# EspressoSystems/Push-CDN

Measured on AMD Instinct MI355X. Metric: broadcast_msgs_per_sec, higher is better.
Workload: dtype uint8; 1 GPU; model=gpu-broker-mesh, payload_bytes=1024, subscribers_total=10000, subscribers_per_broker=10000, topics=8, mode=broadcast, population=all, drops=0, parallelism=single-broker, global_batch=256, seq_len=1024

## Files before the change

### csrc/common/tick_geom.h

```cpp
#pragma once

#include <stdint.h>

#define K2B_BLK 32

#define DENSE_THREADS 256
#define DENSE_MAX_V 8
#define DENSE_GROUP 8
struct DenseGeom { int32_t n_chunks; int32_t chunk_units; };
static inline DenseGeom dense_geom(int32_t units_per_rec) {
    const int32_t cap = DENSE_THREADS * DENSE_MAX_V;
    const int32_t image = units_per_rec * K2B_BLK;
    DenseGeom g;
    g.n_chunks = (image + cap - 1) / cap;
    g.chunk_units = ((image + g.n_chunks - 1) / g.n_chunks + 63) & ~63;
    return g;
}
static inline int64_t dense_grid_x(int32_t n_users, int32_t group, int32_t n_chunks) {
    return ((int64_t)n_users + group - 1) / group * n_chunks;
}

static inline int64_t k2b_blocks(int64_t M) { return (M + K2B_BLK - 1) / K2B_BLK; }
static inline int64_t uniform_tick_scratch64(int64_t M, int64_t W, int64_t units_per_rec) {
    return 4 * M + W * M + k2b_blocks(M) * W * 64 + W * 64 + 2 * M * units_per_rec;
}
static inline int64_t uniform_tick_scratch32(int64_t M, int64_t W) {
    return 3 * M + 3 * k2b_blocks(M) * W * 64 + 2 * W * 64;
}
```

### csrc/gpu_bindings.cpp

```cpp

#include <torch/extension.h>
#include <ATen/hip/HIPContext.h>
#include <c10/core/DeviceGuard.h>
#include <hip/hip_runtime.h>

#include <cstdint>

#include "hip/bls_kernels.h"
#include "hip/dataplane.h"

template <typename T> struct Stored { using type = T; };
template <> struct Stored<uint64_t> { using type = int64_t; };
template <> struct Stored<uint32_t> { using type = int32_t; };
template <> struct Stored<PairRec> { using type = int32_t; };

struct Shape { int64_t dim = -1, rows = -1, cols = -1; };
static constexpr Shape vec() { return {1, -1, -1}; }
static constexpr Shape mat(int64_t rows = -1, int64_t cols = -1) { return {2, rows, cols}; }

class Op {
public:
    enum Where { kDevice, kPinnedHost };

    explicit Op(const char* name) : name_(name) {}
// ... 650 lines not shown
    t.M = a.i32(M, "M");
    t.hash_seed = hash_seed;
    t.sub_bitmap = a.ptr<uint64_t>(sub_bitmap, "sub_bitmap", 0, mat(256, -1));
    const int64_t W = sub_bitmap.size(1);
    t.W = a.i32(W, "W");
    t.n_users = a.i32(n_users, "n_users", 0, W * 64);
    a.ring_bytes(ring_bytes);
    t.ring_bytes = ring_bytes;
    t.ring_wpos = a.ptr<uint64_t>(ring_wpos, "ring_wpos", n_users);
    t.pairs = a.pairs(pairs);
    t.capacity = a.i32(pairs.size(0), "pair capacity");
    t.drops = a.ptr<uint32_t>(drops, "drops", 1);
    t.n_pairs = a.ptr<int32_t>(n_pairs, "n_pairs", 1);
    t.n_sparse = a.ptr<int32_t>(n_sparse, "n_sparse", 1);
    t.scratch64 = a.ptr<int64_t>(scratch64, "scratch64", uniform_tick_scratch64(M, W, rec / 16));
    t.scratch32 = a.ptr<int32_t>(scratch32, "scratch32", uniform_tick_scratch32(M, W));
    t.egress = a.ptr<uint8_t>(egress, "egress", n_users * ring_bytes);
    t.seq_base = (uint32_t)seq_base;
    t.nt = nt != 0;
    t.dense = dense != 0;
    TORCH_CHECK(buf.numel() >= M * uniform_len, a.name(), ": buf has ", buf.numel(),
                " bytes, shorter than M = ", M, " messages of uniform_len = ", uniform_len);
    check_flat_shape(pairs, rec / 16);
    TORCH_CHECK(M * (rec / 16) < (int64_t(1) << 31)
                && dense_grid_x(t.n_users, DENSE_GROUP, dense_geom((int32_t)(rec / 16)).n_chunks)
                       * k2b_blocks(M) < (int64_t(1) << 31),
                a.name(), ": batch too large for the dense fan-out");
    TORCH_CHECK((uintptr_t)t.scratch64 % 16 == 0, a.name(), ": scratch64 must be 16-byte aligned");
    hipStream_t s = a.begin();
    if (M == 0) return;
    launch_tick_uniform_broadcast(&t, s);
    a.launched();
}

std::vector<int64_t> uniform_tick_scratch_sizes(int64_t M, int64_t W, int64_t rec) {
    return {uniform_tick_scratch64(M, W, rec / 16), uniform_tick_scratch32(M, W)};
}

void drain_cursors(torch::Tensor ring_wpos, torch::Tensor staging, torch::Tensor host) {
    Op a("drain_cursors");
    int64_t* wpos = a.ptr<int64_t>(ring_wpos, "ring_wpos");
    const int32_t n = a.i32(ring_wpos.numel(), "cursor count");
    int64_t* st = a.ptr<int64_t>(staging, "staging", n);
    int64_t* h = a.ptr<int64_t>(host, "host", n, {}, Op::kPinnedHost);
    hipStream_t s = a.begin();
    if (n == 0) return;
    launch_drain_cursors(wpos, st, n, s);
    a.launched();
    a.check(hipMemcpyAsync(h, st, (size_t)n * 8, hipMemcpyDeviceToHost, s), "copy");
    a.check(hipStreamSynchronize(s), "sync");
}

PYBIND11_MODULE(TORCH_EXTENSION_NAME, m) {
    m.def("tick_uniform_broadcast", &tick_uniform_broadcast,
          "fused uniform broadcast tick: K4, K2a, K2b tiles, dense + sparse fan-out");
    m.def("uniform_tick_scratch_sizes", &uniform_tick_scratch_sizes,
          "(int64, int32) scratch elements tick_uniform_broadcast needs for (M, W, rec)");
    m.def("drain_cursors", &drain_cursors,
          "fused drain: cursors -> pinned host buffer, cursors zeroed, stream synchronised",
          py::call_guard<py::gil_scoped_release>());
    m.def("topic_mask_origin_t", &topic_mask_origin_t,
          "K2a transposed with per-message origin: remote-origin rows keep user bits only");
    m.def("emit_direct_peers", &emit_direct_peers,
          "K5b with peer recipient slots (owner -(p+2) -> ring n_users+p, local origin only)");
    m.def("direct_apply", &direct_apply,
          "K6: batched DirectMap upserts/deletes on the device table");
    m.def("parse_batch", &parse_batch, "K4: on-device capnp parse of a message batch",
          py::arg("buf"), py::arg("offsets"), py::arg("hash_seed") = 0);
    m.def("topic_mask", &topic_mask, "K2a: per-message subscriber mask");
    m.def("assign_emit", &assign_emit, "K2b: per-user FIFO ring assignment + pair list");
    m.def("fanout", &fanout, "K3: N-way payload fan-out into egress rings");
    m.def("direct_lookup", &direct_lookup, "K5: batched direct-route hash probe");
    m.def("apply_subs", &apply_subs, "K2c: apply subscribe/unsubscribe batch to bitmap");
    m.def("bls_verify_batch", &bls_verify_batch, "K1: batched BLS-over-BN254 verification");
    m.def("compact_rings", &compact_rings,
          "K7: gather used egress-ring prefixes into one staging buffer");
    m.def("precompute_g2_lines", &precompute_g2_lines,
          "fixed-g2 Miller line coefficients for K1 v2 (once per process)");
    m.def("bls_verify_batch2", &bls_verify_batch2,
          "K1 v2: 2-lane Fp2-decomposed batched BLS verification");
    m.def("bls_verify_batch_wave", &bls_verify_batch_wave,
          "K1 v3: wave-batched product verification (shared final exp, "
          "exact per-item fallback)");
    m.def("hash_to_g1_batch", &hash_to_g1_batch, "K1 helper: batched hash-to-G1");
    m.def("fanout_wave", &fanout_wave, "K3v2: wave-per-pair fan-out (nt flag, device count)");
    m.def("fanout_ref", &fanout_ref,
          "K3r: fan-out with by-reference records at or above ref_threshold");
    m.def("fanout_flat2", &fanout_flat2, "K3v4: flat fan-out, seq from base, capacity clamp");
    m.def("fanout_flat3", &fanout_flat3, "K3v5: graph-capturable (device seq counter)");
    m.def("seq_advance", &seq_advance, "bump the device seq counter (inside the graph)");
    m.def("topic_mask_t", &topic_mask_t, "K2a transposed: mask[W][M]");
    m.def("emit_direct", &emit_direct,
          "K5b: on-device direct-delivery pair emission (no host sync)");
    m.def("assign_emit_fused_t", &assign_emit_fused_t,
          "K2b fused on transposed mask (wave-aggregated claims, uniform-rec fast path)");
    m.def("assign_emit_blocks_t", &assign_emit_blocks_t,
          "K2b block-parallel (P1 count / P2 bases / P3 emit) for uniform records");
}
```

### csrc/hip/dataplane.hip

```cpp

#include <hip/hip_runtime.h>
#include <stdint.h>

#include "../common/divmagic.h"
#include "dataplane.h"

#define WAVE 64
#ifndef CDN_CHECK
#define CDN_CHECK 1
#endif

#define RING_ALIGN 16ull
__host__ __device__ inline uint64_t ring_rec(int32_t len) {
    return ((uint64_t)len + 16 + (RING_ALIGN - 1)) & ~(RING_ALIGN - 1);
}

typedef unsigned int cdn_v4u __attribute__((ext_vector_type(4)));
template <int NT>
__device__ __forceinline__ void store16(void* dst, cdn_v4u v) {
    if (NT) __builtin_nontemporal_store(v, (cdn_v4u*)dst);
    else *(cdn_v4u*)dst = v;
}

__device__ __forceinline__ void store_pair(PairRec* p, int32_t u, int32_t m, int64_t d) {
// ... 2 lines not shown
    store16<0>(p, v);
}

__host__ __device__ inline uint64_t fnv1a64(const uint8_t* data, uint32_t len,
                                            uint64_t seed = 0) {
    uint64_t h = 0xcbf29ce484222325ull ^ seed;
    for (uint32_t i = 0; i < len; ++i) {
        h ^= (uint64_t)data[i];
        h *= 0x100000001b3ull;
    }
    return h;
}


__device__ inline uint64_t ld_u64(const uint8_t* p) {
    uint64_t v;
    memcpy(&v, p, 8);
    return v;
}

__device__ inline bool read_struct_ptr(const uint8_t* seg, int64_t nwords, int64_t pw,
                                       int64_t* tgt, int32_t* dw, int32_t* ptrw) {
    if (pw < 0 || pw >= nwords) return false;
    uint64_t v = ld_u64(seg + pw * 8);
    if (v == 0 || (v & 3) != 0) return false;
    int64_t b = (v >> 2) & 0x3fffffff;
    if (b & 0x20000000) b -= 0x40000000;
    int32_t d = (v >> 32) & 0xffff;
    int32_t p = (v >> 48) & 0xffff;
    int64_t t = pw + 1 + b;
    if (t < 0 || t + d + p > nwords) return false;
    *tgt = t; *dw = d; *ptrw = p;
    return true;
}

__device__ inline bool read_byte_list(const uint8_t* seg, int64_t nwords, int64_t pw,
                                      int64_t* off, int32_t* len) {
    if (pw < 0 || pw >= nwords) return false;
    uint64_t v = ld_u64(seg + pw * 8);
    if (v == 0) { *off = pw; *len = 0; return true; }
    if ((v & 3) != 1) return false;
    int64_t b = (v >> 2) & 0x3fffffff;
    if (b & 0x20000000) b -= 0x40000000;
    uint32_t code = (v >> 32) & 7;
    int64_t count = (v >> 35) & 0x1fffffff;
    if (code != 2) return false;
    int64_t t = pw + 1 + b;
    if (t < 0 || t * 8 + count > nwords * 8) return false;
    *off = t * 8;
    *len = (int32_t)count;
    return true;
}

extern "C" __global__ void k4_parse_batch(
    const uint8_t* __restrict__ buf,
    const int64_t* __restrict__ offsets,
    int32_t M, uint64_t hash_seed, ParseOut out)
{
    int i = blockIdx.x * blockDim.x + threadIdx.x;
    if (i >= M) return;
    out.disc[i] = -1;
    out.payload_off[i] = 0; out.payload_len[i] = 0;
    out.topics_off[i] = 0;  out.topics_cnt[i] = 0;
    out.recip_hash[i] = 0;  out.timestamp[i] = 0;
    int64_t o_poff = 0, o_toff = 0, o_ts = 0;
    uint64_t o_rhash = 0;
    int32_t o_plen = 0, o_tcnt = 0;

    int64_t beg = offsets[i], end = offsets[i + 1];
    if (end - beg < 8 + 8) return;
    const uint8_t* p = buf + beg;
    uint32_t seg_m1, nw;
    memcpy(&seg_m1, p, 4); memcpy(&nw, p + 4, 4);
    if (seg_m1 != 0) return;
    if (8 + (int64_t)nw * 8 > end - beg) return;
    const uint8_t* seg = p + 8;
    int64_t nwords = nw;

    int64_t mt; int32_t mdw, mpw;
    if (!read_struct_ptr(seg, nwords, 0, &mt, &mdw, &mpw)) return;
    if (mdw < 1 || mpw < 1) return;
    uint16_t disc;
    memcpy(&disc, seg + mt * 8, 2);
    int64_t up = mt + mdw;

    int64_t seg_base = (seg - buf);

    switch (disc) {
    case 0: {
        int64_t it; int32_t idw, ipw;
        if (!read_struct_ptr(seg, nwords, up, &it, &idw, &ipw)) return;
        if (idw < 1 || ipw < 2) return;
        o_ts = (int64_t)ld_u64(seg + it * 8);
        int64_t ko; int32_t kl;
        if (!read_byte_list(seg, nwords, it + idw, &ko, &kl)) return;
        o_poff = kl ? seg_base + ko : 0;
        o_plen = kl;
        int64_t so; int32_t sl;
        if (!read_byte_list(seg, nwords, it + idw + 1, &so, &sl)) return;
        o_toff = sl ? seg_base + so : 0;
        o_tcnt = sl;
        break;
    }
    case 1: {
        int64_t it; int32_t idw, ipw;
        if (!read_struct_ptr(seg, nwords, up, &it, &idw, &ipw)) return;
        if (idw < 1) return;
        o_ts = (int64_t)ld_u64(seg + it * 8);
        break;
    }
    case 2: {
        int64_t it; int32_t idw, ipw;
        if (!read_struct_ptr(seg, nwords, up, &it, &idw, &ipw)) return;
        if (idw < 1 || ipw < 1) return;
        o_ts = (int64_t)ld_u64(seg + it * 8);
        int64_t co; int32_t cl;
        if (!read_byte_list(seg, nwords, it + idw, &co, &cl)) return;
        o_poff = cl ? seg_base + co : 0; o_plen = cl;
        break;
    }
    case 3: {
        int64_t it; int32_t idw, ipw;
        if (!read_struct_ptr(seg, nwords, up, &it, &idw, &ipw)) return;
        if (ipw < 2) return;
        int64_t ro; int32_t rl;
        if (!read_byte_list(seg, nwords, it + idw, &ro, &rl)) return;
        o_rhash = fnv1a64(seg + ro, rl, hash_seed);
        int64_t mo; int32_t ml;
        if (!read_byte_list(seg, nwords, it + idw + 1, &mo, &ml)) return;
        o_poff = ml ? seg_base + mo : 0; o_plen = ml;
        break;
    }
    case 4: {
        int64_t it; int32_t idw, ipw;
        if (!read_struct_ptr(seg, nwords, up, &it, &idw, &ipw)) return;
        if (ipw < 2) return;
        int64_t to; int32_t tc;
        if (!read_byte_list(seg, nwords, it + idw, &to, &tc)) return;
        o_toff = tc ? seg_base + to : 0; o_tcnt = tc;
        int64_t mo; int32_t ml;
        if (!read_byte_list(seg, nwords, it + idw + 1, &mo, &ml)) return;
        o_poff = ml ? seg_base + mo : 0; o_plen = ml;
        break;
    }
    case 5: case 6: {
        int64_t to; int32_t tc;
        if (!read_byte_list(seg, nwords, up, &to, &tc)) return;
        o_toff = tc ? seg_base + to : 0; o_tcnt = tc;
        break;
    }
    case 7: case 8: {
        int64_t dof; int32_t dl;
        if (!read_byte_list(seg, nwords, up, &dof, &dl)) return;
        o_poff = dl ? seg_base + dof : 0; o_plen = dl;
        break;
    }
    default:
        return;
    }
    out.payload_off[i] = o_poff; out.payload_len[i] = o_plen;
    out.topics_off[i] = o_toff;  out.topics_cnt[i] = o_tcnt;
    out.recip_hash[i] = (int64_t)o_rhash; out.timestamp[i] = o_ts;
    out.disc[i] = (int32_t)disc;
}


__device__ __forceinline__ uint64_t user_bits_of_word(int32_t w, int32_t n_users) {
    const int64_t lo = (int64_t)w * 64;
    if ((int64_t)n_users >= lo + 64) return ~0ull;
    if ((int64_t)n_users <= lo) return 0ull;
    return (1ull << (n_users - lo)) - 1ull;
}

template <bool SINGLE_HOP>
__device__ __forceinline__ uint64_t topic_row_or(
    const uint64_t* __restrict__ sub_bitmap, const uint8_t* __restrict__ buf,
    const int64_t* __restrict__ topics_off, const int32_t* __restrict__ topics_cnt,
    const int32_t* __restrict__ disc, int64_t m, int w, int32_t W,
    const int32_t* __restrict__ origin, int32_t n_users)
{
    uint64_t acc = 0;
    if (disc[m] == 4) {
        const uint8_t* topics = buf + topics_off[m];
        int n = topics_cnt[m];
        for (int t = 0; t < n; ++t) acc |= sub_bitmap[(int64_t)topics[t] * W + w];
        if (SINGLE_HOP && origin[m] != 0) acc &= user_bits_of_word(w, n_users);
    }
    return acc;
}

extern "C" __global__ void k2a_topic_mask(
    const uint64_t* __restrict__ sub_bitmap,
    const uint8_t* __restrict__ buf,
    const int64_t* __restrict__ topics_off,
    const int32_t* __restrict__ topics_cnt,
    const int32_t* __restrict__ disc,
    uint64_t* __restrict__ mask,
    int32_t M, int32_t W)
{
    int64_t idx = (int64_t)blockIdx.x * blockDim.x + threadIdx.x;
    if (idx >= (int64_t)M * W) return;
    int m = idx / W;
    int w = idx % W;
    mask[idx] = topic_row_or<false>(sub_bitmap, buf, topics_off, topics_cnt, disc, m, w, W,
                                    nullptr, 0);
}

extern "C" __global__ void k2b_count(
    const uint64_t* __restrict__ mask,
    int32_t M, int32_t W, int32_t n_users,
    int32_t* __restrict__ counts)
{
    int u = blockIdx.x * blockDim.x + threadIdx.x;
    if (u >= n_users) return;
    int w = u >> 6;
    uint64_t bit = 1ull << (u & 63);
// ... 470 lines not shown
        const int32_t fit = (int32_t)((ring_bytes - wpos) / (uint64_t)uniform_rec);
        uint32_t dropped = 0;
        int emitted = 0;
        const int64_t dst_base = (int64_t)u * ring_bytes + (int64_t)wpos;
        for (int m = 0; m < M; ++m) {
            if (!(col[m] & bit)) continue;
            const bool ok = (emitted < fit) && (slot < capacity);
            if (!ok) {
                if (slot < capacity) { store_pair(pairs + slot, -1, m, 0); slot++; }
                dropped++;
                continue;
            }
            store_pair(pairs + slot, u, m, dst_base + (int64_t)emitted * uniform_rec);
            slot++;
            emitted++;
        }
        ring_wpos[u] = wpos + (uint64_t)emitted * uniform_rec;
        if (dropped) atomicAdd(drops, dropped);
        return;
    }

    uint64_t wpos = ring_wpos[u];
    uint32_t dropped = 0;
    for (int m = 0; m < M; ++m) {
        if (!(col[m] & bit)) continue;
        int32_t len = payload_len[m];
        uint64_t rec = ring_rec(len);
        bool fits_ring = (wpos + rec <= (uint64_t)ring_bytes);
        bool fits_cap = (slot < capacity);
        if (!fits_ring || !fits_cap) {
            if (fits_cap) { store_pair(pairs + slot, -1, m, 0); slot++; }
            dropped++;
            continue;
        }
        store_pair(pairs + slot, u, m, (int64_t)u * ring_bytes + wpos);
        slot++;
        wpos += rec;
    }
    ring_wpos[u] = wpos;
    if (dropped) atomicAdd(drops, dropped);
}

extern "C" {

void launch_k2a_topic_mask_t(const uint64_t* sub_bitmap, const uint8_t* buf,
                             const int64_t* topics_off, const int32_t* topics_cnt,
                             const int32_t* disc, uint64_t* mask_t, int32_t M, int32_t W,
                             hipStream_t s) {
    if (M <= 0) return;
    hipLaunchKernelGGL(k2a_topic_mask_t, k2a_grid(M, W), dim3(K2A_THREADS), 0, s, sub_bitmap,
                       buf, topics_off, topics_cnt, disc, mask_t, M, W);
}


__device__ __forceinline__ void k2b_p1_body(
    const uint64_t* __restrict__ mask_t,
    int32_t M, int32_t W, int32_t NB,
    int32_t* __restrict__ bcount)
{
    const int wave = (blockIdx.x * blockDim.x + threadIdx.x) >> 6;
    if (wave >= W * NB) return;
    const int w = wave / NB, b = wave - (int64_t)(wave / NB) * NB;
    const int lane = threadIdx.x & 63;
    const uint64_t bit = 1ull << lane;
    const uint64_t* col = mask_t + (int64_t)w * M;
    const int m0 = b * K2B_BLK, m1 = min(M, m0 + K2B_BLK);
    int c = 0;
    for (int m = m0; m < m1; ++m) c += (col[m] & bit) ? 1 : 0;
    bcount[(int64_t)b * (W * 64) + (w * 64 + lane)] = c;
}

extern "C" __global__ void k2b_p1_count(
    const uint64_t* __restrict__ mask_t, int32_t M, int32_t W, int32_t NB,
    int32_t* __restrict__ bcount)
{
    k2b_p1_body(mask_t, M, W, NB, bcount);
}

struct K2bUser { int32_t base; int32_t fit; int64_t dst; };

__device__ __forceinline__ K2bUser k2b_p2_body(
    const int32_t* __restrict__ bcount,
    int u, bool active, int32_t W, int32_t NB,
    int64_t ring_bytes, int32_t capacity, int32_t uniform_rec,
    uint64_t* __restrict__ ring_wpos,
    int32_t* __restrict__ n_pairs,
    int32_t* __restrict__ pprefix,
    uint32_t* __restrict__ drops)
{
    const int lane = threadIdx.x & 63;
    int total = 0;
    if (active) {
        for (int b = 0; b < NB; ++b) {
            pprefix[(int64_t)b * (W * 64) + u] = total;
            total += bcount[(int64_t)b * (W * 64) + u];
        }
    }
    K2bUser r{wave_claim_span(total, n_pairs), 0, 0};
    uint32_t dropped = 0;
    if (active) {
        const uint64_t wpos = ring_wpos[u];
        r.fit = (int32_t)((ring_bytes - wpos) / (uint64_t)uniform_rec);
        r.dst = (int64_t)u * ring_bytes + (int64_t)wpos;
        int cap_room = capacity - r.base; if (cap_room < 0) cap_room = 0;
        int emitted = total; if (emitted > r.fit) emitted = r.fit; if (emitted > cap_room) emitted = cap_room;
        ring_wpos[u] = wpos + (uint64_t)emitted * uniform_rec;
        dropped = (uint32_t)(total - emitted);
    }
    for (int d = 1; d < 64; d <<= 1) dropped += __shfl_down(dropped, d);
    if (lane == 0 && dropped) atomicAdd(drops, dropped);
    return r;
}

extern "C" __global__ void k2b_p2_bases(
    const int32_t* __restrict__ bcount,
    int32_t W, int32_t NB, int32_t n_users,
    int64_t ring_bytes, int32_t capacity, int32_t uniform_rec,
    uint64_t* __restrict__ ring_wpos,
    int32_t* __restrict__ n_pairs,
    int32_t* __restrict__ pprefix,
    int32_t* __restrict__ ubase,
    int32_t* __restrict__ ufit,
    int64_t* __restrict__ udst,
    uint32_t* __restrict__ drops)
{
    const int u = blockIdx.x * blockDim.x + threadIdx.x;
    const bool active = u < n_users;
    const K2bUser r = k2b_p2_body(bcount, u, active, W, NB, ring_bytes, capacity, uniform_rec,
                                  ring_wpos, n_pairs, pprefix, drops);
    if (active) {
        ubase[u] = r.base;
        ufit[u] = r.fit;
        udst[u] = r.dst;
    }
}

extern "C" __global__ void k2b_p3_emit(
    const uint64_t* __restrict__ mask_t,
    const int32_t* __restrict__ pprefix,
    const int32_t* __restrict__ ubase,
    const int32_t* __restrict__ ufit,
    const int64_t* __restrict__ udst,
    int32_t M, int32_t W, int32_t NB, int32_t n_users,
    int32_t capacity, int32_t uniform_rec,
    PairRec* __restrict__ pairs)
{
    const int wave = (blockIdx.x * blockDim.x + threadIdx.x) >> 6;
    if (wave >= W * NB) return;
    const int w = wave / NB, b = wave - (int64_t)(wave / NB) * NB;
    const int lane = threadIdx.x & 63;
    const int u = w * 64 + lane;
    if (u >= n_users) return;
    const uint64_t bit = 1ull << lane;
    const uint64_t* col = mask_t + (int64_t)w * M;
    int p = pprefix[(int64_t)b * (W * 64) + u];
    const int base = ubase[u], fit = ufit[u];
    const int64_t dstb = udst[u];
    const int m0 = b * K2B_BLK, m1 = min(M, m0 + K2B_BLK);
    for (int m = m0; m < m1; ++m) {
        if (!(col[m] & bit)) continue;
        const int slot = base + p;
        if (slot < capacity) {
            if (p < fit)
                store_pair(pairs + slot, u, m, dstb + (int64_t)p * uniform_rec);
            else
                store_pair(pairs + slot, -1, m, 0);
        }
        p++;
    }
}

extern "C" void launch_k2b_blocks_t(
    const uint64_t* mask_t, int32_t M, int32_t W, int32_t n_users,
    int64_t ring_bytes, int32_t capacity, int32_t uniform_rec,
    uint64_t* ring_wpos, int32_t* n_pairs,
    int32_t* bcount, int32_t* pprefix, int32_t* ubase, int32_t* ufit, int64_t* udst,
    PairRec* pairs,
    uint32_t* drops, hipStream_t s) {
    if (M <= 0) return;
    const int NB = (M + K2B_BLK - 1) / K2B_BLK;
    const int waves = W * NB;
    const int threads = 256;
    const int blocks_wb = (waves * 64 + threads - 1) / threads;
    const int blocks_u = (n_users + threads - 1) / threads;
    hipLaunchKernelGGL(k2b_p1_count, dim3(blocks_wb), dim3(threads), 0, s,
                       mask_t, M, W, NB, bcount);
    hipLaunchKernelGGL(k2b_p2_bases, dim3(blocks_u), dim3(threads), 0, s,
                       bcount, W, NB, n_users, ring_bytes, capacity, uniform_rec,
                       ring_wpos, n_pairs, pprefix, ubase, ufit, udst, drops);
    hipLaunchKernelGGL(k2b_p3_emit, dim3(blocks_wb), dim3(threads), 0, s,
                       mask_t, pprefix, ubase, ufit, udst, M, W, NB, n_users,
                       capacity, uniform_rec, pairs);
}

void launch_k2b_fused_t(const uint64_t* mask_t, const int32_t* payload_len, int32_t M,
                        int32_t W, int32_t n_users, int64_t ring_bytes, int32_t capacity,
                        int32_t uniform_rec, uint64_t* ring_wpos, int32_t* n_pairs,
                        PairRec* pairs,
                        uint32_t* drops, hipStream_t s) {
    int threads = 256, blocks = (n_users + threads - 1) / threads;
    hipLaunchKernelGGL(k2b_fused_t, dim3(blocks), dim3(threads), 0, s, mask_t, payload_len, M,
                       W, n_users, ring_bytes, capacity, uniform_rec, ring_wpos, n_pairs,
                       pairs, drops);
}

}


__device__ __forceinline__ void k5b_claim_emit(
    int u, int i, int32_t len, int64_t ring_bytes, int32_t capacity,
    uint64_t* __restrict__ ring_wpos, int32_t* __restrict__ n_pairs,
    PairRec* __restrict__ pairs, uint32_t* __restrict__ drops)
{
    uint64_t rec = ring_rec(len);
    int slot = atomicAdd(n_pairs, 1);
    if (slot >= capacity) {
        atomicAdd(drops, 1u);
        return;
    }
    unsigned long long cur = atomicAdd((unsigned long long*)&ring_wpos[u], 0ull);
    while (true) {
        if (cur + rec > (uint64_t)ring_bytes) {
            store_pair(pairs + slot, -1, i, 0);
            atomicAdd(drops, 1u);
            return;
        }
        unsigned long long prev = atomicCAS((unsigned long long*)&ring_wpos[u], cur,
                                            cur + (unsigned long long)rec);
        if (prev == cur) break;
        cur = prev;
    }
    store_pair(pairs + slot, u, i, (int64_t)u * ring_bytes + (int64_t)cur);
}

extern "C" __global__ void k5b_emit_direct(
    const int32_t* __restrict__ disc,
    const int32_t* __restrict__ owner,
    const int64_t* __restrict__ payload_off,
    const int32_t* __restrict__ payload_len,
    int32_t M,
    int64_t ring_bytes, int32_t capacity,
    uint64_t* __restrict__ ring_wpos,
    int32_t* __restrict__ n_pairs,
    PairRec* __restrict__ pairs,
    uint32_t* __restrict__ drops)
{
    int i = blockIdx.x * blockDim.x + threadIdx.x;
// ... 137 lines not shown
                                             __HIP_MEMORY_SCOPE_AGENT);
        if (k == key) { table_vals[slot] = INT32_MIN; return; }
        if (k == 0) return;
    }
}

extern "C" {

void launch_k2a_topic_mask_origin_t(const uint64_t* sub_bitmap, const uint8_t* buf,
                                    const int64_t* topics_off, const int32_t* topics_cnt,
                                    const int32_t* disc, const int32_t* origin,
                                    uint64_t* mask_t, int32_t M, int32_t W, int32_t n_users,
                                    hipStream_t s) {
    if (M <= 0) return;
    hipLaunchKernelGGL(k2a_topic_mask_origin_t, k2a_grid(M, W), dim3(K2A_THREADS), 0, s,
                       sub_bitmap, buf, topics_off, topics_cnt, disc, origin, mask_t, M, W,
                       n_users);
}

void launch_k5b_emit_direct_peers(
    const int32_t* disc, const int32_t* owner, const int32_t* origin,
    const int64_t* payload_off, const int32_t* payload_len, int32_t M, int32_t n_users,
    int32_t n_peers, int64_t ring_bytes, int32_t capacity, uint64_t* ring_wpos,
    int32_t* n_pairs, PairRec* pairs, uint32_t* drops, hipStream_t s) {
    if (M <= 0) return;
    int threads = 256, blocks = (M + threads - 1) / threads;
    hipLaunchKernelGGL(k5b_emit_direct_peers, dim3(blocks), dim3(threads), 0, s, disc, owner,
                       origin, payload_off, payload_len, M, n_users, n_peers, ring_bytes,
                       capacity, ring_wpos, n_pairs, pairs, drops);
}

void launch_k6_direct_apply(uint64_t* table_keys, int32_t* table_vals, int64_t table_size,
                            const uint64_t* up_keys, const int32_t* up_owners, int32_t n_up,
                            const uint64_t* del_keys, int32_t n_del, uint32_t* n_failed,
                            hipStream_t s) {
    const int total = n_up + n_del;
    if (total <= 0) return;
    int threads = 256, blocks = (total + threads - 1) / threads;
    hipLaunchKernelGGL(k6_direct_apply, dim3(blocks), dim3(threads), 0, s, table_keys,
                       table_vals, table_size, up_keys, up_owners, n_up, del_keys, n_del,
                       n_failed);
}

}

extern "C" __global__ void k2b_p1_count_z(
    const uint64_t* __restrict__ mask_t, int32_t M, int32_t W, int32_t NB,
    int32_t* __restrict__ bcount, int32_t* __restrict__ n_pairs, int32_t* __restrict__ n_sparse)
{
    if (blockIdx.x == 0 && threadIdx.x == 0) { *n_pairs = 0; *n_sparse = 0; }
    k2b_p1_body(mask_t, M, W, NB, bcount);
}

extern "C" __global__ void k2b_p2_tiles(
    const int32_t* __restrict__ bcount,
    int32_t M, int32_t W, int32_t NB, int32_t n_users,
    int64_t ring_bytes, int32_t capacity, int32_t uniform_rec, int32_t use_dense,
    uint64_t* __restrict__ ring_wpos,
    int32_t* __restrict__ n_pairs,
    int32_t* __restrict__ n_sparse,
    int32_t* __restrict__ pprefix,
    int32_t* __restrict__ tslot,
    int64_t* __restrict__ tdst,
    int32_t* __restrict__ ulim,
    int32_t* __restrict__ usbase,
    int64_t* __restrict__ udst,
    uint32_t* __restrict__ drops)
{
    const int u = blockIdx.x * blockDim.x + threadIdx.x;
    const bool active = u < n_users;
    const K2bUser r = k2b_p2_body(bcount, u, active, W, NB, ring_bytes, capacity, uniform_rec,
                                  ring_wpos, n_pairs, pprefix, drops);
    int cap_room = capacity - r.base; if (cap_room < 0) cap_room = 0;
    const int lim = r.fit < cap_room ? r.fit : cap_room;
    int n_sp = 0;
    if (active) {
        int p = 0;
        for (int b = 0; b < NB; ++b) {
            const int64_t i = (int64_t)b * (W * 64) + u;
            const int cnt = bcount[i];
            const int nm = min(M - b * K2B_BLK, K2B_BLK);
            const bool dense = use_dense && cnt == nm && p + cnt <= lim;
            tdst[i] = dense ? r.dst + (int64_t)p * uniform_rec : -1;
            tslot[i] = n_sp;
            if (!dense) n_sp += max(0, min(cnt, lim - p));
            p += cnt;
        }
    }
    const int sbase = wave_claim_span(n_sp, n_sparse);
    if (active) {
        ulim[u] = lim;
        usbase[u] = sbase;
        udst[u] = r.dst;
    }
}

extern "C" __global__ void k2b_p3_sparse(
    const uint64_t* __restrict__ mask_t,
    const int32_t* __restrict__ bcount,
    const int32_t* __restrict__ pprefix,
    const int32_t* __restrict__ tslot,
    const int64_t* __restrict__ tdst,
    const int32_t* __restrict__ ulim,
    const int32_t* __restrict__ usbase,
    const int64_t* __restrict__ udst,
    int32_t M, int32_t W, int32_t NB, int32_t n_users, int32_t uniform_rec,
    PairRec* __restrict__ pairs)
{
    const int wave = (blockIdx.x * blockDim.x + threadIdx.x) >> 6;
    if (wave >= W * NB) return;
    const int w = wave / NB, b = wave - (wave / NB) * NB;
    const int lane = threadIdx.x & 63;
    const int u = w * 64 + lane;
    int p0 = 0, lim = 0, slot0 = 0;
    int64_t dstb = 0;
    bool sparse = false;
    if (u < n_users) {
        const int64_t i = (int64_t)b * (W * 64) + u;
        p0 = pprefix[i];
        lim = ulim[u];
        sparse = tdst[i] < 0 && bcount[i] > 0 && p0 < lim;
        slot0 = usbase[u] + tslot[i];
        dstb = udst[u];
    }
    unsigned long long todo = __ballot(sparse);
    if (!todo) return;
    const int m0 = b * K2B_BLK, nm = min(M - m0, K2B_BLK);
    const uint64_t word = lane < nm ? mask_t[(int64_t)w * M + m0 + lane] : 0ull;
    while (todo) {
        const int j = __ffsll((long long)todo) - 1;
        todo &= todo - 1;
        const int jp0 = __shfl(p0, j), jlim = __shfl(lim, j), jslot = __shfl(slot0, j);
        const int64_t jdst = ((int64_t)__shfl((int)(dstb >> 32), j) << 32)
                             | (uint32_t)__shfl((int)dstb, j);
        const bool bit = (word >> j) & 1ull;
        const unsigned long long mb = __ballot(bit);
        const int rank = __popcll(mb & ((1ull << lane) - 1ull));
        const int p = jp0 + rank;
        if (bit && p < jlim)
            store_pair(pairs + jslot + rank, w * 64 + j, m0 + lane,
                       jdst + (int64_t)p * uniform_rec);
    }
}

extern "C" __global__ void k3d_image(
    const uint8_t* __restrict__ buf,
    const int64_t* __restrict__ offsets,
    int32_t M, int32_t units_per_rec, uint32_t div_magic, int32_t div_shift,
    int32_t uniform_len, uint32_t seq_base,
    cdn_v4u* __restrict__ image)
{
    const uint32_t i = blockIdx.x * blockDim.x + threadIdx.x;
    if (i >= (uint32_t)(M * units_per_rec)) return;
    const int m = (int)(((uint64_t)i * div_magic) >> div_shift);
    const int q = (int)i - m * units_per_rec;
    image[i] = q == 0 ? cdn_v4u{(uint32_t)uniform_len, seq_base + (uint32_t)m, 0u, 0u}
                      : payload_unit(buf + offsets[m], (q - 1) * 16, uniform_len);
}

__global__ void __launch_bounds__(DENSE_THREADS) k3_fanout_dense(
    const cdn_v4u* __restrict__ image,
    const int64_t* __restrict__ tdst,
    int32_t M, int32_t NB, int32_t users64, int32_t n_users, int32_t units_per_rec,
    int32_t n_chunks, int32_t chunk_units, int32_t group,
    uint8_t* __restrict__ egress)
{
    const int per_group = NB * n_chunks;
    const int g = blockIdx.x / per_group, bc = blockIdx.x - g * per_group;
    const int b = bc / n_chunks, c = bc - b * n_chunks;
    const int m0 = b * K2B_BLK, nm = min(M - m0, K2B_BLK);
    const int lo = c * chunk_units + (int)threadIdx.x;
    const int hi = min(nm * units_per_rec, (c + 1) * chunk_units);
    if (lo >= hi) return;
    const cdn_v4u* __restrict__ img = image + (size_t)m0 * units_per_rec;
    cdn_v4u v[DENSE_MAX_V];
    #pragma unroll
    for (int k = 0; k < DENSE_MAX_V; ++k) {
        const int unit = lo + k * DENSE_THREADS;
        v[k] = unit < hi ? img[unit] : cdn_v4u{0u, 0u, 0u, 0u};
    }
    const int64_t* __restrict__ trow = tdst + (int64_t)b * users64;
    const int u1 = min(n_users, (g + 1) * group);
    for (int u = g * group; u < u1; ++u) {
        const int64_t d = trow[u];
        if (d < 0) continue;
        uint8_t* dst = egress + d + (size_t)lo * 16;
        #pragma unroll
        for (int k = 0; k < DENSE_MAX_V; ++k)
            if (lo + k * DENSE_THREADS < hi)
                store16<0>(dst + (size_t)k * (DENSE_THREADS * 16), v[k]);
    }
}

extern "C" __global__ void k_drain_cursors(int64_t* __restrict__ ring_wpos,
                                           int64_t* __restrict__ staging, int32_t n)
{
    const int i = blockIdx.x * blockDim.x + threadIdx.x;
    if (i >= n) return;
    staging[i] = ring_wpos[i];
    ring_wpos[i] = 0;
}

extern "C" {

void launch_tick_uniform_broadcast(const UniformTick* t, hipStream_t s) {
    const int32_t M = t->M, W = t->W;
    if (M <= 0) return;
    const int32_t NB = (int32_t)k2b_blocks(M);
    const int64_t U = (int64_t)W * 64, T = (int64_t)NB * U;
    const int32_t units = t->rec / 16;
    int64_t* p64 = t->scratch64;
    cdn_v4u* image = (cdn_v4u*)p64;  p64 += 2 * (int64_t)M * units;
    int64_t* payload_off = p64;  p64 += M;
    int64_t* topics_off = p64;   p64 += M;
    int64_t* recip_hash = p64;   p64 += M;
    int64_t* timestamp = p64;    p64 += M;
    uint64_t* mask_t = (uint64_t*)p64;  p64 += (int64_t)W * M;
    int64_t* tdst = p64;         p64 += T;
    int64_t* udst = p64;
    int32_t* p32 = t->scratch32;
    int32_t* disc = p32;         p32 += M;
    int32_t* payload_len = p32;  p32 += M;
    int32_t* topics_cnt = p32;   p32 += M;
    int32_t* bcount = p32;       p32 += T;
    int32_t* pprefix = p32;      p32 += T;
    int32_t* tslot = p32;        p32 += T;
    int32_t* ulim = p32;         p32 += U;
    int32_t* usbase = p32;

    launch_k4_parse(t->buf, t->offsets, M, t->hash_seed,
                    ParseOut{disc, payload_off, payload_len, topics_off, topics_cnt,
                             (uint64_t*)recip_hash, (uint64_t*)timestamp}, s);
    launch_k2a_topic_mask_t(t->sub_bitmap, t->buf, topics_off, topics_cnt, disc, mask_t, M, W, s);

    const int threads = 256;
    const int blocks_wb = (W * NB * 64 + threads - 1) / threads;
    const int blocks_u = (t->n_users + threads - 1) / threads;
    hipLaunchKernelGGL(k2b_p1_count_z, dim3(blocks_wb), dim3(threads), 0, s, mask_t, M, W, NB,
                       bcount, t->n_pairs, t->n_sparse);
    hipLaunchKernelGGL(k2b_p2_tiles, dim3(blocks_u), dim3(threads), 0, s, bcount, M, W, NB,
                       t->n_users, t->ring_bytes, t->capacity, t->rec, t->dense ? 1 : 0,
                       t->ring_wpos, t->n_pairs, t->n_sparse, pprefix, tslot, tdst, ulim, usbase,
                       udst, t->drops);
    hipLaunchKernelGGL(k2b_p3_sparse, dim3(blocks_wb), dim3(threads), 0, s, mask_t, bcount,
                       pprefix, tslot, tdst, ulim, usbase, udst, M, W, NB, t->n_users, t->rec,
                       t->pairs);
    if (t->dense) {
        const DenseGeom geo = dense_geom(units);
        uint32_t dm; int32_t dsh;
        u32_div_magic(units, &dm, &dsh);
        hipLaunchKernelGGL(k3d_image, dim3((M * units + threads - 1) / threads), dim3(threads),
                           0, s, t->buf, t->offsets, M, units, dm, dsh, t->uniform_len,
                           t->seq_base, image);
        const dim3 grid((uint32_t)(dense_grid_x(t->n_users, DENSE_GROUP, geo.n_chunks) * NB));
        hipLaunchKernelGGL(k3_fanout_dense, grid, dim3(DENSE_THREADS), 0, s, image, tdst, M, NB,
                           (int32_t)U, t->n_users, units, geo.n_chunks, geo.chunk_units,
                           DENSE_GROUP, t->egress);
    }
    launch_flat<false>(t->buf, t->offsets, payload_len, t->pairs, t->seq_base, nullptr,
                       t->n_sparse, t->capacity, units, t->uniform_len, t->egress, t->nt, 0, s);
}

void launch_drain_cursors(int64_t* ring_wpos, int64_t* staging, int32_t n, hipStream_t s) {
    if (n <= 0) return;
    hipLaunchKernelGGL(k_drain_cursors, dim3((n + 255) / 256), dim3(256), 0, s, ring_wpos,
                       staging, n);
}

}
```

Measured before the change: 429,700 msgs/s.

## Fuse routing stages into one per-word LDS kernel and merge parse with image build

Replaces the separate topic-mask, count, tile-assign and sparse-pair kernels with a single per-word workgroup kernel. It keeps the mask column, counts, prefixes and slots in LDS using narrow 8/16-bit types when the batch fits (M ≤ 3584). It also merges the parse and dense-image kernels into one prologue launch that zeroes the counters. The aim is to cut kernel launches and global-memory round trips for intermediate arrays. In exchange, only W workgroups run the routing (157 for 10k users), so parallelism drops and LDS use limits occupancy.

```diff
diff --git a/csrc/common/tick_geom.h b/csrc/common/tick_geom.h
--- a/csrc/common/tick_geom.h
+++ b/csrc/common/tick_geom.h
@@ -27,3 +27,26 @@
 static inline int64_t uniform_tick_scratch32(int64_t M, int64_t W) {
     return 3 * M + 3 * k2b_blocks(M) * W * 64 + 2 * W * 64;
 }
+
+#define ROUTE_THREADS 256
+struct RouteLds { int32_t mask, udst, ulim, usbase, pprefix, tslot, bcount, bytes; };
+constexpr RouteLds route_lds(int32_t M) {
+    const int32_t tiles = (M + K2B_BLK - 1) / K2B_BLK * 64;
+    RouteLds l{};
+    l.mask = 0;
+    l.udst = l.mask + 8 * M;
+    l.ulim = l.udst + 8 * 64;
+    l.usbase = l.ulim + 4 * 64;
+    l.pprefix = l.usbase + 4 * 64;
+    l.tslot = l.pprefix + 2 * tiles;
+    l.bcount = l.tslot + 2 * tiles;
+    l.bytes = l.bcount + tiles;
+    return l;
+}
+#define ROUTE_MAX_M 3584
+static_assert(route_lds(ROUTE_MAX_M).bytes <= 64 * 1024, "route kernel LDS exceeds a workgroup's 64 KiB");
+static_assert(route_lds(ROUTE_MAX_M + 1).bytes > 64 * 1024, "ROUTE_MAX_M is not the largest batch that fits");
+static_assert(ROUTE_MAX_M >= 2048, "the 8-GPU bench routes 8 x 256 gathered messages per tick");
+static_assert(ROUTE_MAX_M <= 65535 && K2B_BLK <= 255, "prefixes are 16-bit, tile counts 8-bit");
+static_assert(route_lds(33).udst % 8 == 0 && route_lds(33).ulim % 4 == 0 && route_lds(33).pprefix % 2 == 0,
+              "route kernel LDS arrays are aligned to their element types");
diff --git a/csrc/gpu_bindings.cpp b/csrc/gpu_bindings.cpp
--- a/csrc/gpu_bindings.cpp
+++ b/csrc/gpu_bindings.cpp
@@ -726,6 +726,7 @@
 }
 
 PYBIND11_MODULE(TORCH_EXTENSION_NAME, m) {
+    m.attr("_ROUTE_MAX_M") = py::int_(ROUTE_MAX_M);
     m.def("tick_uniform_broadcast", &tick_uniform_broadcast,
           "fused uniform broadcast tick: K4, K2a, K2b tiles, dense + sparse fan-out");
     m.def("uniform_tick_scratch_sizes", &uniform_tick_scratch_sizes,
diff --git a/csrc/hip/dataplane.hip b/csrc/hip/dataplane.hip
--- a/csrc/hip/dataplane.hip
+++ b/csrc/hip/dataplane.hip
@@ -78,12 +78,11 @@
     return true;
 }
 
-extern "C" __global__ void k4_parse_batch(
+__device__ __forceinline__ void k4_parse_body(
     const uint8_t* __restrict__ buf,
     const int64_t* __restrict__ offsets,
-    int32_t M, uint64_t hash_seed, ParseOut out)
-{
-    int i = blockIdx.x * blockDim.x + threadIdx.x;
+    int32_t M, uint64_t hash_seed, const ParseOut& out, int i)
+{
     if (i >= M) return;
     out.disc[i] = -1;
     out.payload_off[i] = 0; out.payload_len[i] = 0;
@@ -188,6 +187,14 @@
     out.topics_off[i] = o_toff;  out.topics_cnt[i] = o_tcnt;
     out.recip_hash[i] = (int64_t)o_rhash; out.timestamp[i] = o_ts;
     out.disc[i] = (int32_t)disc;
+}
+
+extern "C" __global__ void k4_parse_batch(
+    const uint8_t* __restrict__ buf,
+    const int64_t* __restrict__ offsets,
+    int32_t M, uint64_t hash_seed, ParseOut out)
+{
+    k4_parse_body(buf, offsets, M, hash_seed, out, blockIdx.x * blockDim.x + threadIdx.x);
 }
 
 
@@ -764,6 +771,18 @@
                        buf, topics_off, topics_cnt, disc, mask_t, M, W);
 }
 
+}
+
+
+
+__device__ __forceinline__ int k2b_tile_count(const uint64_t* __restrict__ wcol, int32_t M, int b)
+{
+    const uint64_t bit = 1ull << (threadIdx.x & 63);
+    const int m0 = b * K2B_BLK, m1 = min(M, m0 + K2B_BLK);
+    int c = 0;
+    for (int m = m0; m < m1; ++m) c += (wcol[m] & bit) ? 1 : 0;
+    return c;
+}
 
 __device__ __forceinline__ void k2b_p1_body(
     const uint64_t* __restrict__ mask_t,
@@ -774,12 +793,7 @@
     if (wave >= W * NB) return;
     const int w = wave / NB, b = wave - (int64_t)(wave / NB) * NB;
     const int lane = threadIdx.x & 63;
-    const uint64_t bit = 1ull << lane;
-    const uint64_t* col = mask_t + (int64_t)w * M;
-    const int m0 = b * K2B_BLK, m1 = min(M, m0 + K2B_BLK);
-    int c = 0;
-    for (int m = m0; m < m1; ++m) c += (col[m] & bit) ? 1 : 0;
-    bcount[(int64_t)b * (W * 64) + (w * 64 + lane)] = c;
+    bcount[(int64_t)b * (W * 64) + (w * 64 + lane)] = k2b_tile_count(mask_t + (int64_t)w * M, M, b);
 }
 
 extern "C" __global__ void k2b_p1_count(
@@ -791,21 +805,22 @@
 
 struct K2bUser { int32_t base; int32_t fit; int64_t dst; };
 
+template <class Cnt, class Pre>
 __device__ __forceinline__ K2bUser k2b_p2_body(
-    const int32_t* __restrict__ bcount,
-    int u, bool active, int32_t W, int32_t NB,
+    const Cnt* __restrict__ bcount,
+    int u, bool active, int32_t stride, int col, int32_t NB,
     int64_t ring_bytes, int32_t capacity, int32_t uniform_rec,
     uint64_t* __restrict__ ring_wpos,
     int32_t* __restrict__ n_pairs,
-    int32_t* __restrict__ pprefix,
+    Pre* __restrict__ pprefix,
     uint32_t* __restrict__ drops)
 {
     const int lane = threadIdx.x & 63;
     int total = 0;
     if (active) {
         for (int b = 0; b < NB; ++b) {
-            pprefix[(int64_t)b * (W * 64) + u] = total;
-            total += bcount[(int64_t)b * (W * 64) + u];
+            pprefix[(int64_t)b * stride + col] = (Pre)total;
+            total += bcount[(int64_t)b * stride + col];
         }
     }
     K2bUser r{wave_claim_span(total, n_pairs), 0, 0};
@@ -838,8 +853,8 @@
 {
     const int u = blockIdx.x * blockDim.x + threadIdx.x;
     const bool active = u < n_users;
-    const K2bUser r = k2b_p2_body(bcount, u, active, W, NB, ring_bytes, capacity, uniform_rec,
-                                  ring_wpos, n_pairs, pprefix, drops);
+    const K2bUser r = k2b_p2_body(bcount, u, active, W * 64, u, NB, ring_bytes, capacity,
+                                  uniform_rec, ring_wpos, n_pairs, pprefix, drops);
     if (active) {
         ubase[u] = r.base;
         ufit[u] = r.fit;
@@ -905,6 +920,8 @@
                        capacity, uniform_rec, pairs);
 }
 
+extern "C" {
+
 void launch_k2b_fused_t(const uint64_t* mask_t, const int32_t* payload_len, int32_t M,
                         int32_t W, int32_t n_users, int64_t ring_bytes, int32_t capacity,
                         int32_t uniform_rec, uint64_t* ring_wpos, int32_t* n_pairs,
@@ -1148,6 +1165,42 @@
     k2b_p1_body(mask_t, M, W, NB, bcount);
 }
 
+struct K2bTiles { int32_t lim; int32_t sbase; int64_t dst; };
+
+template <class Cnt, class Pre, class Slot>
+__device__ __forceinline__ K2bTiles k2b_tiles_body(
+    const Cnt* __restrict__ bcount,
+    int u, bool active, int32_t stride, int col, int32_t M, int32_t W, int32_t NB,
+    int64_t ring_bytes, int32_t capacity, int32_t uniform_rec, int32_t use_dense,
+    uint64_t* __restrict__ ring_wpos,
+    int32_t* __restrict__ n_pairs,
+    int32_t* __restrict__ n_sparse,
+    Pre* __restrict__ pprefix,
+    Slot* __restrict__ tslot,
+    int64_t* __restrict__ tdst,
+    uint32_t* __restrict__ drops)
+{
+    const K2bUser r = k2b_p2_body(bcount, u, active, stride, col, NB, ring_bytes, capacity,
+                                  uniform_rec, ring_wpos, n_pairs, pprefix, drops);
+    int cap_room = capacity - r.base; if (cap_room < 0) cap_room = 0;
+    const int lim = r.fit < cap_room ? r.fit : cap_room;
+    int n_sp = 0;
+    if (active) {
+        int p = 0;
+        for (int b = 0; b < NB; ++b) {
+            const int64_t i = (int64_t)b * stride + col;
+            const int cnt = bcount[i];
+            const int nm = min(M - b * K2B_BLK, K2B_BLK);
+            const bool dense = use_dense && cnt == nm && p + cnt <= lim;
+            tdst[(int64_t)b * (W * 64) + u] = dense ? r.dst + (int64_t)p * uniform_rec : -1;
+            tslot[i] = (Slot)n_sp;
+            if (!dense) n_sp += max(0, min(cnt, lim - p));
+            p += cnt;
+        }
+    }
+    return K2bTiles{lim, wave_claim_span(n_sp, n_sparse), r.dst};
+}
+
 extern "C" __global__ void k2b_p2_tiles(
     const int32_t* __restrict__ bcount,
     int32_t M, int32_t W, int32_t NB, int32_t n_users,
@@ -1165,64 +1218,47 @@
 {
     const int u = blockIdx.x * blockDim.x + threadIdx.x;
     const bool active = u < n_users;
-    const K2bUser r = k2b_p2_body(bcount, u, active, W, NB, ring_bytes, capacity, uniform_rec,
-                                  ring_wpos, n_pairs, pprefix, drops);
-    int cap_room = capacity - r.base; if (cap_room < 0) cap_room = 0;
-    const int lim = r.fit < cap_room ? r.fit : cap_room;
-    int n_sp = 0;
+    const K2bTiles r = k2b_tiles_body(bcount, u, active, W * 64, u, M, W, NB, ring_bytes, capacity,
+                                      uniform_rec, use_dense, ring_wpos, n_pairs, n_sparse,
+                                      pprefix, tslot, tdst, drops);
     if (active) {
-        int p = 0;
-        for (int b = 0; b < NB; ++b) {
-            const int64_t i = (int64_t)b * (W * 64) + u;
-            const int cnt = bcount[i];
-            const int nm = min(M - b * K2B_BLK, K2B_BLK);
-            const bool dense = use_dense && cnt == nm && p + cnt <= lim;
-            tdst[i] = dense ? r.dst + (int64_t)p * uniform_rec : -1;
-            tslot[i] = n_sp;
-            if (!dense) n_sp += max(0, min(cnt, lim - p));
-            p += cnt;
-        }
-    }
-    const int sbase = wave_claim_span(n_sp, n_sparse);
-    if (active) {
-        ulim[u] = lim;
-        usbase[u] = sbase;
+        ulim[u] = r.lim;
+        usbase[u] = r.sbase;
         udst[u] = r.dst;
     }
 }
 
-extern "C" __global__ void k2b_p3_sparse(
-    const uint64_t* __restrict__ mask_t,
-    const int32_t* __restrict__ bcount,
-    const int32_t* __restrict__ pprefix,
-    const int32_t* __restrict__ tslot,
+template <class Cnt, class Pre, class Slot>
+__device__ __forceinline__ void k2b_p3_sparse_body(
+    const uint64_t* __restrict__ wcol,
+    const Cnt* __restrict__ bcount,
+    const Pre* __restrict__ pprefix,
+    const Slot* __restrict__ tslot,
     const int64_t* __restrict__ tdst,
     const int32_t* __restrict__ ulim,
     const int32_t* __restrict__ usbase,
     const int64_t* __restrict__ udst,
-    int32_t M, int32_t W, int32_t NB, int32_t n_users, int32_t uniform_rec,
+    int w, int b, int32_t stride, int col,
+    int32_t M, int32_t W, int32_t n_users, int32_t uniform_rec,
     PairRec* __restrict__ pairs)
 {
-    const int wave = (blockIdx.x * blockDim.x + threadIdx.x) >> 6;
-    if (wave >= W * NB) return;
-    const int w = wave / NB, b = wave - (wave / NB) * NB;
     const int lane = threadIdx.x & 63;
     const int u = w * 64 + lane;
     int p0 = 0, lim = 0, slot0 = 0;
     int64_t dstb = 0;
     bool sparse = false;
     if (u < n_users) {
-        const int64_t i = (int64_t)b * (W * 64) + u;
+        const int64_t i = (int64_t)b * stride + col;
         p0 = pprefix[i];
-        lim = ulim[u];
-        sparse = tdst[i] < 0 && bcount[i] > 0 && p0 < lim;
-        slot0 = usbase[u] + tslot[i];
-        dstb = udst[u];
+        lim = ulim[col];
+        sparse = tdst[(int64_t)b * (W * 64) + u] < 0 && bcount[i] > 0 && p0 < lim;
+        slot0 = usbase[col] + tslot[i];
+        dstb = udst[col];
     }
     unsigned long long todo = __ballot(sparse);
     if (!todo) return;
     const int m0 = b * K2B_BLK, nm = min(M - m0, K2B_BLK);
-    const uint64_t word = lane < nm ? mask_t[(int64_t)w * M + m0 + lane] : 0ull;
+    const uint64_t word = lane < nm ? wcol[m0 + lane] : 0ull;
     while (todo) {
         const int j = __ffsll((long long)todo) - 1;
         todo &= todo - 1;
@@ -1239,19 +1275,107 @@
     }
 }
 
-extern "C" __global__ void k3d_image(
+extern "C" __global__ void k2b_p3_sparse(
+    const uint64_t* __restrict__ mask_t,
+    const int32_t* __restrict__ bcount,
+    const int32_t* __restrict__ pprefix,
+    const int32_t* __restrict__ tslot,
+    const int64_t* __restrict__ tdst,
+    const int32_t* __restrict__ ulim,
+    const int32_t* __restrict__ usbase,
+    const int64_t* __restrict__ udst,
+    int32_t M, int32_t W, int32_t NB, int32_t n_users, int32_t uniform_rec,
+    PairRec* __restrict__ pairs)
+{
+    const int wave = (blockIdx.x * blockDim.x + threadIdx.x) >> 6;
+    if (wave >= W * NB) return;
+    const int w = wave / NB, b = wave - (wave / NB) * NB;
+    k2b_p3_sparse_body(mask_t + (int64_t)w * M, bcount, pprefix, tslot, tdst, ulim, usbase, udst,
+                       w, b, W * 64, w * 64 + (int)(threadIdx.x & 63), M, W, n_users,
+                       uniform_rec, pairs);
+}
+
+extern "C" __global__ void __launch_bounds__(ROUTE_THREADS) k_route_word(
+    const uint64_t* __restrict__ sub_bitmap,
+    const uint8_t* __restrict__ buf,
+    const int64_t* __restrict__ topics_off,
+    const int32_t* __restrict__ topics_cnt,
+    const int32_t* __restrict__ disc,
+    int32_t M, int32_t W, int32_t NB, int32_t n_users,
+    int64_t ring_bytes, int32_t capacity, int32_t uniform_rec, int32_t use_dense,
+    uint64_t* __restrict__ ring_wpos,
+    int32_t* __restrict__ n_pairs,
+    int32_t* __restrict__ n_sparse,
+    int64_t* __restrict__ tdst,
+    PairRec* __restrict__ pairs,
+    uint32_t* __restrict__ drops)
+{
+    extern __shared__ __attribute__((aligned(16))) uint8_t route_smem[];
+    const RouteLds l = route_lds(M);
+    uint64_t* wcol = (uint64_t*)(route_smem + l.mask);
+    int64_t* udst = (int64_t*)(route_smem + l.udst);
+    int32_t* ulim = (int32_t*)(route_smem + l.ulim);
+    int32_t* usbase = (int32_t*)(route_smem + l.usbase);
+    uint16_t* pprefix = (uint16_t*)(route_smem + l.pprefix);
+    uint16_t* tslot = (uint16_t*)(route_smem + l.tslot);
+    uint8_t* bcount = route_smem + l.bcount;
+
+    const int w = blockIdx.x;
+    const int lane = threadIdx.x & 63, wave = threadIdx.x >> 6, n_waves = blockDim.x >> 6;
+    const int u = w * 64 + lane;
+
+    for (int m = threadIdx.x; m < M; m += blockDim.x)
+        wcol[m] = topic_row_or<false>(sub_bitmap, buf, topics_off, topics_cnt, disc, m, w, W,
+                                      nullptr, 0);
+    __syncthreads();
+    for (int b = wave; b < NB; b += n_waves)
+        bcount[b * 64 + lane] = (uint8_t)k2b_tile_count(wcol, M, b);
+    __syncthreads();
+    if (wave == 0) {
+        const bool active = u < n_users;
+        const K2bTiles r = k2b_tiles_body(bcount, u, active, 64, lane, M, W, NB, ring_bytes,
+                                          capacity, uniform_rec, use_dense, ring_wpos, n_pairs,
+                                          n_sparse, pprefix, tslot, tdst, drops);
+        ulim[lane] = r.lim;
+        usbase[lane] = r.sbase;
+        udst[lane] = r.dst;
+    }
+    __syncthreads();
+    for (int b = wave; b < NB; b += n_waves)
+        k2b_p3_sparse_body(wcol, bcount, pprefix, tslot, tdst, ulim, usbase, udst, w, b, 64, lane,
+                           M, W, n_users, uniform_rec, pairs);
+}
+
+__device__ __forceinline__ void k3d_image_body(
     const uint8_t* __restrict__ buf,
     const int64_t* __restrict__ offsets,
     int32_t M, int32_t units_per_rec, uint32_t div_magic, int32_t div_shift,
     int32_t uniform_len, uint32_t seq_base,
-    cdn_v4u* __restrict__ image)
-{
-    const uint32_t i = blockIdx.x * blockDim.x + threadIdx.x;
+    cdn_v4u* __restrict__ image,
+    uint32_t i)
+{
     if (i >= (uint32_t)(M * units_per_rec)) return;
     const int m = (int)(((uint64_t)i * div_magic) >> div_shift);
     const int q = (int)i - m * units_per_rec;
     image[i] = q == 0 ? cdn_v4u{(uint32_t)uniform_len, seq_base + (uint32_t)m, 0u, 0u}
                       : payload_unit(buf + offsets[m], (q - 1) * 16, uniform_len);
+}
+
+extern "C" __global__ void __launch_bounds__(256) k_tick_prologue(
+    const uint8_t* __restrict__ buf,
+    const int64_t* __restrict__ offsets,
+    int32_t M, uint64_t hash_seed, ParseOut out, int32_t parse_blocks,
+    int32_t units_per_rec, uint32_t div_magic, int32_t div_shift,
+    int32_t uniform_len, uint32_t seq_base,
+    cdn_v4u* __restrict__ image,
+    int32_t* __restrict__ n_pairs, int32_t* __restrict__ n_sparse)
+{
+    if (blockIdx.x == 0 && threadIdx.x == 0) { *n_pairs = 0; *n_sparse = 0; }
+    if ((int32_t)blockIdx.x < parse_blocks)
+        k4_parse_body(buf, offsets, M, hash_seed, out, blockIdx.x * blockDim.x + threadIdx.x);
+    else
+        k3d_image_body(buf, offsets, M, units_per_rec, div_magic, div_shift, uniform_len, seq_base,
+                       image, (blockIdx.x - parse_blocks) * blockDim.x + threadIdx.x);
 }
 
 __global__ void __launch_bounds__(DENSE_THREADS) k3_fanout_dense(
@@ -1324,30 +1448,41 @@
     int32_t* ulim = p32;         p32 += U;
     int32_t* usbase = p32;
 
-    launch_k4_parse(t->buf, t->offsets, M, t->hash_seed,
-                    ParseOut{disc, payload_off, payload_len, topics_off, topics_cnt,
-                             (uint64_t*)recip_hash, (uint64_t*)timestamp}, s);
-    launch_k2a_topic_mask_t(t->sub_bitmap, t->buf, topics_off, topics_cnt, disc, mask_t, M, W, s);
-
     const int threads = 256;
-    const int blocks_wb = (W * NB * 64 + threads - 1) / threads;
-    const int blocks_u = (t->n_users + threads - 1) / threads;
-    hipLaunchKernelGGL(k2b_p1_count_z, dim3(blocks_wb), dim3(threads), 0, s, mask_t, M, W, NB,
-                       bcount, t->n_pairs, t->n_sparse);
-    hipLaunchKernelGGL(k2b_p2_tiles, dim3(blocks_u), dim3(threads), 0, s, bcount, M, W, NB,
-                       t->n_users, t->ring_bytes, t->capacity, t->rec, t->dense ? 1 : 0,
-                       t->ring_wpos, t->n_pairs, t->n_sparse, pprefix, tslot, tdst, ulim, usbase,
-                       udst, t->drops);
-    hipLaunchKernelGGL(k2b_p3_sparse, dim3(blocks_wb), dim3(threads), 0, s, mask_t, bcount,
-                       pprefix, tslot, tdst, ulim, usbase, udst, M, W, NB, t->n_users, t->rec,
-                       t->pairs);
+    const int parse_blocks = (M + threads - 1) / threads;
+    const int image_blocks = t->dense ? (M * units + threads - 1) / threads : 0;
+    uint32_t dm; int32_t dsh;
+    u32_div_magic(units, &dm, &dsh);
+    hipLaunchKernelGGL(k_tick_prologue, dim3(parse_blocks + image_blocks), dim3(threads), 0, s,
+                       t->buf, t->offsets, M, t->hash_seed,
+                       ParseOut{disc, payload_off, payload_len, topics_off, topics_cnt,
+                                (uint64_t*)recip_hash, (uint64_t*)timestamp},
+                       parse_blocks, units, dm, dsh, t->uniform_len, t->seq_base, image,
+                       t->n_pairs, t->n_sparse);
+
+    if (M <= ROUTE_MAX_M) {
+        hipLaunchKernelGGL(k_route_word, dim3(W), dim3(ROUTE_THREADS), route_lds(M).bytes, s,
+                           t->sub_bitmap, t->buf, topics_off, topics_cnt, disc, M, W, NB,
+                           t->n_users, t->ring_bytes, t->capacity, t->rec, t->dense ? 1 : 0,
+                           t->ring_wpos, t->n_pairs, t->n_sparse, tdst, t->pairs, t->drops);
+    } else {
+        launch_k2a_topic_mask_t(t->sub_bitmap, t->buf, topics_off, topics_cnt, disc, mask_t, M, W,
+                                s);
+        const int blocks_wb = (W * NB * 64 + threads - 1) / threads;
+        const int blocks_u = (t->n_users + threads - 1) / threads;
+        hipLaunchKernelGGL(k2b_p1_count_z, dim3(blocks_wb), dim3(threads), 0, s, mask_t, M, W, NB,
+                           bcount, t->n_pairs, t->n_sparse);
+        hipLaunchKernelGGL(k2b_p2_tiles, dim3(blocks_u), dim3(threads), 0, s, bcount, M, W, NB,
+                           t->n_users, t->ring_bytes, t->capacity, t->rec, t->dense ? 1 : 0,
+                           t->ring_wpos, t->n_pairs, t->n_sparse, pprefix, tslot, tdst, ulim,
+                           usbase, udst, t->drops);
+        hipLaunchKernelGGL(k2b_p3_sparse, dim3(blocks_wb), dim3(threads), 0, s, mask_t, bcount,
+                           pprefix, tslot, tdst, ulim, usbase, udst, M, W, NB, t->n_users, t->rec,
+                           t->pairs);
+    }
+
     if (t->dense) {
         const DenseGeom geo = dense_geom(units);
-        uint32_t dm; int32_t dsh;
-        u32_div_magic(units, &dm, &dsh);
-        hipLaunchKernelGGL(k3d_image, dim3((M * units + threads - 1) / threads), dim3(threads),
-                           0, s, t->buf, t->offsets, M, units, dm, dsh, t->uniform_len,
-                           t->seq_base, image);
         const dim3 grid((uint32_t)(dense_grid_x(t->n_users, DENSE_GROUP, geo.n_chunks) * NB));
         hipLaunchKernelGGL(k3_fanout_dense, grid, dim3(DENSE_THREADS), 0, s, image, tdst, M, NB,
                            (int32_t)U, t->n_users, units, geo.n_chunks, geo.chunk_units,
```

Measured after the change: 454,200 msgs/s (median of 6 runs). 5.7% higher.
